# aptx4869lm/4DCapture-FPV

Hardware: AMD Instinct MI355X
Metric: frames/sec global-opt (fixed iters), 1024f clip/500k-pt scene; Chamfer GB/s (higher is better)
Workload: dtype f32; 1 GPU; BASELINE config 3: 1024-frame clip, 500000-pt scene, 500 contact verts, 500 Adam iterations (phase split 0.8), full loss; frames sharded over 1 GPU(s); frames=1024, scene_points=500000, contact_verts=500, iters=500, body_verts=10475, lbs_weights_per_vertex=4

## Files before the change

4dcapture-fpv_amd/csrc/fdc_chamfer.h:

```cpp
#pragma once
#include <hip/hip_runtime.h>
#include <stdlib.h>

#include <atomic>

#include "fdc_forms.h"
#include "fdc_math.h"

namespace fdc {

constexpr int NN_TILE = 1024;

struct NNTarget {
    const float4* pts;
    int n;
    const float4* bounds;
    const float4* sbounds;
    const float4* qbounds;
    const int* inv_perm;
    const uint4* frags;
    const float4* centers;
};


// ... 966 lines not shown
    scan(bc);
    if (T.centers) {
        float bm = INFINITY;
        int bc2 = -1;
        auto centre = [&](int c) {
            const float4 cc = T.centers[c];
            const float dx = x - cc.x, dy = y - cc.y, dz = z - cc.z;
            const float m = __builtin_amdgcn_sqrtf(fmaf(dz, dz, fmaf(dy, dy, dx * dx))) + cc.w;
            if (m < bm) { bm = m; bc2 = c; }
        };
        if (T.sbounds) {
            const int nsuper = (nchunk + ST4_SUPER - 1) / ST4_SUPER;
            for (int sb = 0; sb < nsuper; ++sb) {
                if (!(box_d2(T.sbounds[2 * sb], T.sbounds[2 * sb + 1], x, y, z) < bm * bm)) continue;
                for (int c = sb * ST4_SUPER; c < min(nchunk, (sb + 1) * ST4_SUPER); ++c) centre(c);
            }
        } else
            for (int c = 0; c < nchunk; ++c) centre(c);
        if (bc2 >= 0 && bc2 != bc && bm * bm < bd) scan(bc2);
    }
    seed[qi] = bi;
    seedpt[qi] = bp;
}

__global__ void nn_records_gather_kernel(const int* __restrict__ idx, int nq, const float4* __restrict__ scene, const int* __restrict__ inv_perm,
                                         float4* __restrict__ seedpt) {
    const int qi = blockIdx.x * blockDim.x + threadIdx.x;
    if (qi >= nq) return;
    const int j = idx[qi];
    if (j < 0) return;
    const float4 p = scene[j];
    seedpt[qi] = make_float4(p.x, p.y, p.z, __int_as_float(inv_perm[j]));
}

__global__ void nn_combine_kernel(const float* __restrict__ pd, const int* __restrict__ pi, int nsplit, int nq,
                                  float* __restrict__ dist, int* __restrict__ idx) {
    int qi = blockIdx.x * blockDim.x + threadIdx.x;
    if (qi >= nq) return;
    float best = INFINITY;
    int bi = -1;
    for (int s = 0; s < nsplit; ++s) {
        float d = pd[(size_t)s * nq + qi];
        int j = pi[(size_t)s * nq + qi];
        if (j >= 0 && (bi < 0 || nn_better(d, j, best, bi))) { best = d; bi = j; }
    }
    dist[qi] = best;
    idx[qi] = bi;
}

__global__ void pack_points_kernel(const float* __restrict__ xyz, int n, float4* __restrict__ out) {
    int i = blockIdx.x * blockDim.x + threadIdx.x;
    if (i >= n) return;
    out[i] = make_float4(xyz[3 * (size_t)i], xyz[3 * (size_t)i + 1], xyz[3 * (size_t)i + 2], __int_as_float(i));
}

__global__ void pack_points_batched_kernel(const float* __restrict__ xyz, long long stride, int n, float4* __restrict__ out) {
    int i = blockIdx.x * blockDim.x + threadIdx.x;
    if (i >= n) return;
    const float* const p = xyz + (size_t)blockIdx.y * stride + 3 * (size_t)i;
    out[(size_t)blockIdx.y * n + i] = make_float4(p[0], p[1], p[2], __int_as_float(i));
}
__global__ void nn_combine_batched_kernel(const float* __restrict__ pd, const int* __restrict__ pi, int nsplit, int nq,
                                          float* __restrict__ dist, int* __restrict__ idx) {
    int qi = blockIdx.x * blockDim.x + threadIdx.x;
    if (qi >= nq) return;
    const size_t bb = blockIdx.y;
    pd += bb * nsplit * nq; pi += bb * nsplit * nq;
    float best = INFINITY;
    int bi = -1;
    for (int s = 0; s < nsplit; ++s) {
        float d = pd[(size_t)s * nq + qi];
        int j = pi[(size_t)s * nq + qi];
        if (j >= 0 && (bi < 0 || nn_better(d, j, best, bi))) { best = d; bi = j; }
    }
    dist[bb * nq + qi] = best;
    idx[bb * nq + qi] = bi;
}

__global__ void nn_grad_kernel(const float* __restrict__ q, const float4* __restrict__ tgt, const float* __restrict__ g,
                               const int* __restrict__ idx, int nq, float* __restrict__ gq) {
    int qi = blockIdx.x * blockDim.x + threadIdx.x;
    if (qi >= nq) return;
    int j = idx[qi];
    float gg = 2.f * g[qi];
    float4 p = j >= 0 ? tgt[j] : make_float4(0, 0, 0, 0);
    gq[3 * (size_t)qi] = j >= 0 ? gg * (q[3 * (size_t)qi] - p.x) : 0.f;
    gq[3 * (size_t)qi + 1] = j >= 0 ? gg * (q[3 * (size_t)qi + 1] - p.y) : 0.f;
    gq[3 * (size_t)qi + 2] = j >= 0 ? gg * (q[3 * (size_t)qi + 2] - p.z) : 0.f;
}

inline std::atomic<int>& nn_mode_ref() {
    static std::atomic<int> mode{0};
    return mode;
}

__global__ __launch_bounds__(1024) void nn_order_kernel(const int* __restrict__ work, int n, const int* __restrict__ prev,
                                                        int* __restrict__ order) {
    __shared__ int cnt[16][256], base[256];
    const int tid = threadIdx.x, w = tid >> 6;
    for (int e = tid; e < 16 * 256; e += 1024) (&cnt[0][0])[e] = 0;
    __syncthreads();
    for (int i = tid; i < n; i += 1024) atomicAdd(&cnt[w][255 - min(max(work[i], 0), 255)], 1);
    __syncthreads();
    if (tid < 256) {
        int run = 0;
        for (int k = 0; k < 16; ++k) { const int t = cnt[k][tid]; cnt[k][tid] = run; run += t; }
        base[tid] = run;
    }
    __syncthreads();
    if (tid < 64) {
        const int a = base[4 * tid], b = base[4 * tid + 1], c = base[4 * tid + 2], d = base[4 * tid + 3];
        int s = a + b + c + d, incl = s;
        for (int off = 1; off < 64; off <<= 1) { const int t = __shfl_up(incl, off, 64); if (tid >= off) incl += t; }
        const int ex = incl - s;
        base[4 * tid] = ex; base[4 * tid + 1] = ex + a; base[4 * tid + 2] = ex + a + b; base[4 * tid + 3] = ex + a + b + c;
    }
    __syncthreads();
    for (int i = tid; i < n; i += 1024) {
        const int k = 255 - min(max(work[i], 0), 255);
        order[base[k] + atomicAdd(&cnt[w][k], 1)] = prev ? prev[i] : i;
    }
}
struct NNOrder {
    bool on = false;
    int sorted_groups = 0;
    int cur = 0;
    int age = 0;
    int every = 32;
    int* qbuf = nullptr;
    int perm_n = 0;
    int perm_mode = 0;
    int n_kept = 0, n_permuted = 0, n_rebuilds = 0;
    int n_box[4] = {0, 0, 0, 0};
};
static inline size_t nn_query_order_ints(int nq);
static inline hipError_t nn_query_order(const float4* seedpt, int nq, int* qbuf, int* hdr, int groups, hipStream_t st);

static inline NNCache nn_stream_args(const NNCache* cache, NNOrder* ord, int groups, int wpg, int nq, const int* seed, const int* idx,
                                     const float4* seedpt, bool seed_missing) {
    NNCache nc = cache ? *cache : NNCache{nullptr, nullptr, nullptr, 0.f};
    const bool ordered = ord != nullptr && ord->on && nc.hdr != nullptr && ord->every > 0 && wpg == 1;
    nc.order_mode = !ordered ? 0 : (ord->sorted_groups == groups ? 2 + ord->cur : 1);
    const bool qorder = ordered && ord->qbuf != nullptr && ord->perm_mode != 1;
    nc.perm = qorder && ord->perm_n == nq ? ord->qbuf : nullptr;
    nc.keep = nc.keep && wpg == 1 && seedpt != nullptr && seed != nullptr && seed == idx && !seed_missing;
    if (ord) { ord->n_kept += nc.keep ? 1 : 0; ord->n_permuted += nc.perm ? 1 : 0; }
    if (ord && wpg == 1) ++ord->n_box[nc.box_lanes == 2 ? 1 : nc.box_lanes == 4 ? 2 : nc.box_lanes == 8 ? 3 : 0];
    return nc;
}
static inline hipError_t nn_stream_upkeep(const NNCache& nc, NNOrder* ord, int groups, int wpg, int nq, const float4* seedpt, bool seed_missing,
                                          hipStream_t st) {
    const bool ordered = ord != nullptr && ord->on && nc.hdr != nullptr && ord->every > 0 && wpg == 1;
    const bool qorder = ordered && ord->qbuf != nullptr && ord->perm_mode != 1;
    const bool resort = ordered && (ord->sorted_groups != groups || ++ord->age >= ord->every);
    if (qorder && ord->perm_mode == 0 && (ord->perm_n != nq || seed_missing || (resort && ord->sorted_groups == groups))) {
        const hipError_t e = nn_query_order(seedpt, nq, ord->qbuf, nc.hdr, groups, st);
        if (e != hipSuccess) return e;
        ord->perm_n = nq;
        ord->sorted_groups = 0;
        ord->age = 0;
        ++ord->n_rebuilds;
    } else if (resort) {
        const bool had = nc.order_mode >= 2;
        const int nxt = had ? 1 - ord->cur : 0;
        hipLaunchKernelGGL(nn_order_kernel, dim3(1), dim3(1024), 0, st, (const int*)(nc.hdr + 4 * groups), groups,
                           had ? (const int*)(nc.hdr + (5 + ord->cur) * groups) : (const int*)nullptr, nc.hdr + (5 + nxt) * groups);
        ord->cur = nxt;
        ord->sorted_groups = groups;
        ord->age = 0;
    }
    return hipSuccess;
}

static inline hipError_t nn_search(const float* q, int nq, const NNTarget& T, float* dist, int* idx, float* pd, int* pi,
                                   int nsplit, hipStream_t st, const int* seed = nullptr, bool seed_missing = false,
                                   float4* seedpt = nullptr, bool* seedpt_written = nullptr, const NNCache* cache = nullptr,
                                   NNOrder* ord = nullptr) {
    if (seedpt_written) *seedpt_written = false;
    if (nq <= 0) return hipSuccess;
    const NNPlan pl = plan_nn_search(nq, T.n, seed != nullptr && T.bounds != nullptr, T.frags != nullptr, seedpt != nullptr && seed == idx, nsplit,
                                     nn_mode_ref(), proc_switches());
    const dim3 grid(pl.grid), block(pl.block);
    note_form(form_name(pl.form));
    if (pl.wpg) {
        if (seed_missing)
            hipLaunchKernelGGL(nn_seed_kernel, dim3((nq + 255) / 256), dim3(256), 0, st, q, nq, T, idx, seedpt);
        if (seedpt_written) *seedpt_written = true;
        {
            const int groups = pl.groups, wpg = pl.wpg;
            const NNCache nc = nn_stream_args(cache, ord, groups, wpg, nq, seed, idx, seedpt, seed_missing);
            if (wpg == 4) hipLaunchKernelGGL((nn_stream4_kernel<4>), grid, block, 0, st, q, nq, T, seed, seedpt, dist, idx, nc, NNNoSegs{});
            else if (wpg == 2) hipLaunchKernelGGL((nn_stream4_kernel<2>), grid, block, 0, st, q, nq, T, seed, seedpt, dist, idx, nc, NNNoSegs{});
            else hipLaunchKernelGGL((nn_stream4_kernel<1, 1>), grid, block, 0, st, q, nq, T, seed, seedpt, dist, idx, nc, NNNoSegs{});
            const hipError_t e = nn_stream_upkeep(nc, ord, groups, wpg, nq, seedpt, seed_missing, st);
            if (e != hipSuccess) return e;
        }
        return hipGetLastError();
    }
    if (pl.form == F_NN_MFMA && pl.nq_blocks == 2) hipLaunchKernelGGL((nn_mfma_kernel<2>), grid, block, 0, st, q, nq, T, nsplit, seed, pd, pi, 0LL, 0LL);
    else if (pl.form == F_NN_MFMA) hipLaunchKernelGGL((nn_mfma_kernel<4>), grid, block, 0, st, q, nq, T, nsplit, seed, pd, pi, 0LL, 0LL);
    else hipLaunchKernelGGL((nn_direct_kernel<2>), grid, block, 0, st, q, nq, T, nsplit, pd, pi, 0LL, 0LL);
    hipLaunchKernelGGL(nn_combine_kernel, dim3((nq + 255) / 256), dim3(256), 0, st, pd, pi, nsplit, nq, dist, idx);
    return hipGetLastError();
}

struct NNSegSearch { const float* q; int nq; NNTarget T; float* dist; int* idx; float4* seedpt; NNCache cache; NNOrder* ord; bool seed_missing; };
static inline hipError_t nn_search_segments(const NNSegPlan& pl, const NNSegSearch* sg, int nseg, hipStream_t st) {
    if (!pl.one_launch || nseg < 1 || nseg > NN_MAX_SEGS || pl.grid_y != nseg) return hipErrorInvalidValue;
    note_form(pl.name);
    NNSegs a{};
    for (int s = 0; s < nseg; ++s) {
        const NNSegSearch& g = sg[s];
        const int groups = (g.nq + 31) / 32;
        if (g.nq <= 0 || groups > pl.grid_x) return hipErrorInvalidValue;
        if (g.seed_missing)
            hipLaunchKernelGGL(nn_seed_kernel, dim3((g.nq + 255) / 256), dim3(256), 0, st, g.q, g.nq, g.T, g.idx, g.seedpt);
        NNSeg& d = a.s[s];
        d.q = g.q; d.nq = g.nq; d.groups = groups; d.T = g.T; d.idx = g.idx; d.seedpt = g.seedpt; d.dist = g.dist;
        d.cache = nn_stream_args(&g.cache, g.ord, groups, 1, g.nq, g.idx, g.idx, g.seedpt, g.seed_missing);
    }
    hipLaunchKernelGGL((nn_stream4_kernel<1, 1, true>), dim3(pl.grid_x, nseg), dim3(pl.block), 0, st, (const float*)nullptr, 0, NNTarget{},
                       (const int*)nullptr, (float4*)nullptr, (float*)nullptr, (int*)nullptr, NNCache{nullptr, nullptr, nullptr, 0.f}, a);
    for (int s = 0; s < nseg; ++s) {
        const NNSegSearch& g = sg[s];
        const hipError_t e = nn_stream_upkeep(a.s[s].cache, g.ord, a.s[s].groups, 1, g.nq, g.seedpt, g.seed_missing, st);
        if (e != hipSuccess) return e;
    }
    return hipGetLastError();
}

static inline hipError_t nn_search_batched(const NNBatchPlan& pl, const float* q, long long qs, int nq, const float* tgt, long long ts, int nt,
                                           int B, float4* pk, float* dist, int* idx, float* pd, int* pi, hipStream_t st) {
    note_form(pl.name);
    const long long pks = ts == 0 ? 0 : nt;
    for (int b0 = 0; b0 < B; b0 += NN_MAX_GRID_Y) {
        const int nb = std::min(B - b0, NN_MAX_GRID_Y);
        const float* const qb = q + (size_t)b0 * qs;
        float4* const pkb = pk + (size_t)b0 * pks;
        float* const pdb = pd + (size_t)b0 * pl.nsplit * nq;
        int* const pib = pi + (size_t)b0 * pl.nsplit * nq;
        if (ts != 0 || b0 == 0)
            hipLaunchKernelGGL(pack_points_batched_kernel, dim3((nt + 255) / 256, ts == 0 ? 1 : nb), dim3(256), 0, st, tgt + (size_t)b0 * ts, ts, nt, pkb);
        const NNTarget T{pkb, nt, nullptr, nullptr, nullptr, nullptr, nullptr, nullptr};
        const dim3 grid(pl.grid_x, nb), block(pl.block);
        if (pl.mfma) hipLaunchKernelGGL((nn_mfma_kernel<4, true>), grid, block, 0, st, qb, nq, T, pl.nsplit, (const int*)nullptr, pdb, pib, qs, pks);
        else hipLaunchKernelGGL((nn_direct_kernel<2, true>), grid, block, 0, st, qb, nq, T, pl.nsplit, pdb, pib, qs, pks);
        hipLaunchKernelGGL(nn_combine_batched_kernel, dim3((nq + 255) / 256, nb), dim3(256), 0, st, pdb, pib, pl.nsplit, nq,
                           dist + (size_t)b0 * nq, idx + (size_t)b0 * nq);
    }
    return hipGetLastError();
}

}
```

4dcapture-fpv_amd/csrc/fdc_chamfer_bwd.h:

```cpp
#pragma once
#include <hip/hip_runtime.h>

#include "fdc_scene.h"

namespace fdc {

static_assert(SC_RS_TILE == QS_TILE, "the histogram and the scatter kernel cut the keys into the same tiles");

constexpr long long CB_MAX_SORT = 0x7fffffffLL - 2 * QS_TILE;

static inline int cb_blocks(long long n) { return (int)((n + QS_TILE - 1) / QS_TILE); }
static inline int cb_passes(unsigned maxkey) { int p = 1; while (p < 4 && (maxkey >> (8 * p)) != 0u) ++p; return p; }
static inline size_t cb_key_words(long long n) { return 2 * (size_t)n + 256 * (size_t)cb_blocks(n) + 256; }

__global__ __launch_bounds__(256) void cb_keys_kernel(const int* __restrict__ idx, int total, int cnt, int ndest, int per_batch,
                                                      unsigned invalid, unsigned* __restrict__ key, int* __restrict__ val) {
    const long long p = (long long)blockIdx.x * 256 + threadIdx.x;
    if (p >= total) return;
    const int j = idx[p];
    const unsigned b = (unsigned)(p / cnt);
    key[p] = (j >= 0 && j < ndest) ? (per_batch ? b * (unsigned)ndest + (unsigned)j : (unsigned)j) : invalid;
    val[p] = (int)p;
}

static inline hipError_t cb_group(const int* idx, int B, int cnt, int ndest, bool per_batch, unsigned* key, int* val, unsigned* hist,
                                  hipStream_t st, int* buf) {
    const int total = B * cnt, nb = cb_blocks(total);
    const unsigned invalid = per_batch ? (unsigned)B * (unsigned)ndest : (unsigned)ndest;
    unsigned* const tot = hist + 256 * (size_t)nb;
    hipLaunchKernelGGL(cb_keys_kernel, dim3((total + 255) / 256), dim3(256), 0, st, idx, total, cnt, ndest, per_batch ? 1 : 0, invalid, key, val);
    const int passes = cb_passes(invalid);
    for (int pass = 0; pass < passes; ++pass) {
        const size_t a = (size_t)(pass & 1) * total, b = (size_t)((pass & 1) ^ 1) * total;
        hipLaunchKernelGGL(sc_rs_hist_kernel, dim3(nb), dim3(256), 0, st, key + a, total, 8 * pass, hist, nb);
        hipLaunchKernelGGL(nn_qs_rows_kernel, dim3(64), dim3(256), 0, st, hist, nb, tot);
        hipLaunchKernelGGL(nn_qs_scatter_kernel, dim3(nb), dim3(256), 0, st, key + a, val + a, key + b, val + b, total, 8 * pass, hist, tot, nb);
    }
    *buf = passes & 1;
    return hipGetLastError();
}

struct CbSide {
    const float* xo; long long so;
    const float* xs; long long ss;
    int B, no, nsrc;
    const float* g_own; const int* idx_own;
    const float* g_src;
    int reduce;
};
__device__ __forceinline__ void cb_own_term(const CbSide& c, int b0, int d, float acc[3]) {
#pragma clang fp contract(off)
    acc[0] = acc[1] = acc[2] = 0.f;
    if (c.g_own == nullptr) return;
    const int b1 = c.reduce ? c.B : b0 + 1;
    for (int b = b0; b < b1; ++b) {
        const size_t p = (size_t)b * c.no + d;
        const int j = c.idx_own[p];
        if (j < 0 || j >= c.nsrc) continue;
        const float gg = 2.f * c.g_own[p];
        const float* const po = c.xo + (size_t)b * c.so + 3 * (size_t)d;
        const float* const ps = c.xs + (size_t)b * c.ss + 3 * (size_t)j;
#pragma unroll
        for (int k = 0; k < 3; ++k) {
            const float v = gg * (po[k] - ps[k]);
            acc[k] = c.reduce ? acc[k] + v : v;
        }
    }
}
__device__ __forceinline__ void cb_add_term(const CbSide& c, int p, int d, float S[3]) {
#pragma clang fp contract(off)
    const int b = p / c.nsrc, i = p - b * c.nsrc;
    const float gg = 2.f * c.g_src[p];
    const float* const po = c.xo + (size_t)b * c.so + 3 * (size_t)d;
    const float* const ps = c.xs + (size_t)b * c.ss + 3 * (size_t)i;
#pragma unroll
    for (int k = 0; k < 3; ++k) { const float v = gg * (ps[k] - po[k]); S[k] = S[k] + v; }
}
__device__ __forceinline__ void cb_store(float* __restrict__ out, size_t t, const float acc[3], const float S[3]) {
#pragma clang fp contract(off)
#pragma unroll
    for (int k = 0; k < 3; ++k) out[3 * t + k] = acc[k] - S[k];
}

__global__ __launch_bounds__(256) void cb_gather_kernel(CbSide c, const unsigned* __restrict__ skey, const int* __restrict__ sval, int nsorted,
                                                        float* __restrict__ out) {
    const long long t = (long long)blockIdx.x * 256 + threadIdx.x;
    const long long ndest = c.reduce ? (long long)c.no : (long long)c.B * c.no;
    if (t >= ndest) return;
    const int b0 = (int)((unsigned)t / (unsigned)c.no), d = (int)((unsigned)t - (unsigned)b0 * (unsigned)c.no);
    float acc[3], S[3] = {0.f, 0.f, 0.f};
    cb_own_term(c, b0, d, acc);
    if (skey != nullptr) {
        const unsigned want = (unsigned)t;
        int lo = 0, hi = nsorted;
        while (lo < hi) {
            const int mid = lo + ((hi - lo) >> 1);
            if (skey[mid] < want) lo = mid + 1; else hi = mid;
        }
        for (int s = lo; s < nsorted && skey[s] == want; ++s) cb_add_term(c, sval[s], d, S);
    }
    cb_store(out, (size_t)t, acc, S);
}

}
```

4dcapture-fpv_amd/csrc/fdc_forms.h:

```cpp
#pragma once
#include <stddef.h>
#include <stdlib.h>

#include <algorithm>

#include "fdc_clips.h"

#if defined(__HIPCC__)
#define FDC_FORMS_HD __host__ __device__
#else
#define FDC_FORMS_HD
#endif

namespace fdc {

struct FormSwitches {
    int clip_fwd_rows = 336;
    int clip_kgrad_rows = 257;
    int pn_rb2 = 1;
    int pn_nw = 0;
    bool pn_ksw = true;
    bool gemm_split3 = true;
    int nn_stream = -2;
    bool nn_seed = true, nn_cull = true;
// ... 97 lines not shown
    size_t lds = 0;
    size_t max_lds = 0;
    PnMap mp = {};
    bool two_partials = false;
};

inline PanelPlan plan_panel3(int M, int K, int ntile, int nst, int np, const FormSwitches& sw) {
    PanelPlan p;
    const int kpad = (K + 31) & ~31;
    if (kpad > PN3_MAX_K) return p;
    const size_t b_bytes = pn_b_bytes(np, ntile, nst);
    if (b_bytes > (size_t)(16u << 20) && M >= 32 && kpad <= 768) {
        const int nrb = (M + 31) / 32, ncb = (ntile + 7) / 8, cpg = (ncb + 7) / 8;
        p.form = F_PANEL3_WIDE;
        p.cs = std::max(1, std::min(cpg, (256 + 8 * nrb - 1) / (8 * nrb)));
        p.grid = 8 * nrb * p.cs; p.block = 512; p.lds = pn_lds_bytes(np, kpad, 2);
        return p;
    }
    if ((sw.pn_rb2 == 1 || sw.pn_rb2 == 2) && M >= sw.clip_fwd_rows && kpad <= 768 && ntile >= 48) {
        p.form = F_PANEL3_RB2;
        p.grid = 8 * ((M + 31) / 32); p.block = 768; p.lds = pn_lds_bytes(np, kpad, 2);
        return p;
    }
    const int nrb = (M + 15) / 16;
    p.form = F_PANEL3;
    p.nw = 8;
    if (nrb * ((ntile + 7) / 8) < 128 && nrb * ((ntile + 3) / 4) >= 128) p.nw = 4;
    if (sw.pn_nw == 8 || sw.pn_nw == 4 || sw.pn_nw == 2) p.nw = sw.pn_nw;
    p.mp = panel_map(nrb, (ntile + p.nw - 1) / p.nw, (size_t)M * K * 4, b_bytes);
    p.grid = 8 * p.mp.rpg * p.mp.cpg; p.block = 64 * p.nw; p.lds = pn_lds_bytes(np, kpad, 1);
    return p;
}

inline PanelPlan plan_blend_backward(int M, int K, int ntile, int nst, int np, bool may_split, const FormSwitches& sw) {
    PanelPlan p;
    const int kpad = (K + 31) & ~31, nst_all = (K + 31) >> 5;
    if (may_split && (sw.pn_rb2 == 1 || sw.pn_rb2 == 3) && M >= sw.clip_kgrad_rows && ntile <= 32 && nst_all >= 2 &&
        32 * ((nst_all + 1) / 2) <= 768) {
        p.form = F_PANEL3_RB2K;
        p.two_partials = true;
        p.grid = 8 * ((M + 31) / 32); p.block = 512; p.lds = pn_lds_bytes(np, 32 * ((nst_all + 1) / 2), 2);
        return p;
    }
    constexpr int kmin = 1664;
    const bool big_k = (M >= 384 && K >= kmin) || (M >= 192 && K >= kmin + 240);
    if (!big_k && sw.pn_ksw && kpad <= PN3_MAX_K && kpad >= 768 && ((M + 15) / 16) * ((ntile + 7) / 8) < 128) {
        const int nrb = (M + 15) / 16;
        p.form = F_PANEL3_KSW;
        p.T = (nrb * ((ntile + 1) / 2) >= 192 || nrb * ntile > 256) ? 2 : 1;
        p.mp = panel_map(nrb, (ntile + p.T - 1) / p.T, (size_t)M * K * 4, pn_b_bytes(np, ntile, nst));
        p.grid = 8 * p.mp.rpg * p.mp.cpg; p.block = 512; p.lds = pn_lds_bytes(np, kpad, 1);
        p.max_lds = pn_lds_bytes(np, PN3_MAX_K, 1);
        return p;
    }
    if (!big_k && panel_gemm3_fits(K)) return plan_panel3(M, K, ntile, nst, np, sw);
    constexpr int rb = PN3_KLOOP_RB, T = PN3_KLOOP_T;
    p.form = F_PANEL3_KLOOP;
    p.ks = panel_gemm3_kloop_parts(M, ntile);
    p.grid = p.ks * ((ntile + 8 * T - 1) / (8 * T)) * ((M + 16 * rb - 1) / (16 * rb)); p.block = 512;
    p.lds = pn_lds_bytes(np, 32 * PN3_KLOOP_SLAB, rb);
    p.max_lds = 150 * 1024;
    return p;
}

inline size_t blend_skin_lds_bytes(int np, int kfeat, int ja) {
    return pn_lds_bytes(np, (kfeat + 31) & ~31, 2) + (size_t)(32 * ja * 12 + 32 * 12 + 32 * 4 + 2 * 64 * 4 + 3 * 32 * 64) * sizeof(float);
}
struct ContactFwdPlan { Form form = F_SKIN_FWD; int grid = 0, grid_y = 1, block = 0; size_t lds = 0, max_lds = 0; };
inline ContactFwdPlan plan_contact_forward(int nl, int nc, int kfeat, int np, bool blend_done, bool permuted_panel, bool vpack, int K, int ja_hi,
                                           const FormSwitches& sw) {
    ContactFwdPlan p;
    if (!blend_done && sw.fuse_skin && sw.gemm_split3 && permuted_panel && vpack && K <= 4 && nl >= sw.clip_fwd_rows &&
        blend_skin_lds_bytes(np, kfeat, ja_hi) <= (size_t)150 * 1024) {
        p.form = F_BLEND_SKIN_FWD;
        p.grid = 8 * ((nl + 31) / 32); p.block = 768; p.lds = blend_skin_lds_bytes(np, kfeat, ja_hi); p.max_lds = 150 * 1024;
        return p;
    }
    p.grid = (nc + 255) / 256; p.grid_y = nl; p.block = 256;
    return p;
}

constexpr int SKB_VCH = 1024;
constexpr int SKB_ROW = 6;
constexpr int SKS_MAXV = 1024, SKS_MAXNNZ = 6144;
struct SkinBwdPlan {
    Form form = F_NONE;
    int G = 0;
    int vpt = 0, kc = 0;
    int nch = 1;
    int grid = 0, block = 256;
    size_t lds = 0;
    bool ja_rows = false;
};
inline SkinBwdPlan plan_skin_bwd_any(int nrows, int nc, bool mfma_da) {
    SkinBwdPlan p;
    p.lds = mfma_da ? std::max((size_t)std::min(nc, SKB_VCH) * SKB_ROW, (size_t)4 * 64 * 16) * sizeof(float)
                    : (size_t)std::min(nc, SKB_VCH) * 12 * sizeof(float);
    p.grid = nrows;
    if (nc <= SKB_VCH) { p.form = F_SKIN_BWD_FRAME; return p; }
    p.nch = (nc + SKB_VCH - 1) / SKB_VCH;
    p.form = mfma_da ? F_SKIN_BWD_CHUNKS_MFMA : F_SKIN_BWD_CHUNKS_LIST;
    return p;
}
inline SkinBwdPlan plan_contact_skin_bwd(int nl, int nc, int nnz, int K, bool vpack, bool csc_v16, bool aligned16, bool mfma_da, bool skin_vec) {
    const size_t lds_small = (size_t)6 * nc * sizeof(float) + (size_t)nnz * sizeof(float) + (((size_t)nnz * 2 + 15) & ~(size_t)15);
    if (!(nc <= SKS_MAXV && nnz <= SKS_MAXNNZ && lds_small <= 57000)) return plan_skin_bwd_any(nl, nc, mfma_da);
    SkinBwdPlan p;
    p.grid = nl; p.lds = lds_small; p.ja_rows = true;
    const int G = (K + 3) / 4;
    const size_t ldsv = (size_t)9 * nc * sizeof(float) + (size_t)((nnz + 3) & ~3) * sizeof(float) + (size_t)((nnz + 7) & ~7) * 2;
    if (skin_vec && nc <= 512 && G <= 3 && nnz <= 2048 * G && ldsv <= 60000 && (nc & 3) == 0 && vpack && csc_v16 && aligned16) {
        p.form = F_SKIN_BWD_VEC; p.G = G; p.lds = ldsv;
        return p;
    }
    p.form = F_SKIN_BWD_SMALL;
    if (nc <= 512 && nnz <= 2048) { p.vpt = 2; p.kc = 8; }
    else if (nc <= 512) { p.form = F_SKIN_BWD_SMALL_K; p.vpt = 2; p.kc = 24; }
    else if (nnz <= 4096) { p.vpt = 4; p.kc = 16; }
    else { p.vpt = 4; p.kc = 24; }
    return p;
}

#ifndef FDC_MF_CH
#define FDC_MF_CH 512
#endif
constexpr int MF_CH = FDC_MF_CH;
constexpr int MF_MAXCHUNK = 2048;
constexpr FDC_FORMS_HD int nn_split_len(int nt, int nsplit) {
    return ((nt + nsplit - 1) / nsplit + MF_CH - 1) / MF_CH * MF_CH;
}
constexpr int nn_grid_blocks(int qblocks, int nsplit) { return (qblocks + 7) / 8 * 8 * nsplit; }
constexpr bool nn_use_mfma(int nq, int nt, int mode) { return mode == 1 ? false : mode == 2 ? true : (long long)nq * nt >= (1LL << 22); }
inline int nn_pick_nsplit(int nq, int nt, bool culled = false) {
    int qblocks = culled ? (nq + 255) / 256 : (nq + 511) / 512;
    int ns = 1;
    const int target = culled ? 1536 : 1024;
    while (qblocks * ns < target && ns < 64 && nt / (ns * 2) >= 4 * MF_CH) ns *= 2;
    if (!culled && qblocks >= 512 && nt >= 8 * MF_CH) ns = std::max(ns, 2);
    while (nn_split_len(nt, ns) / MF_CH > MF_MAXCHUNK) ns *= 2;
    return ns;
}
constexpr FDC_FORMS_HD int nn_box_lanes(int n, int forced) {
    return (forced == 2 || forced == 4 || forced == 8) ? forced : n <= 8 ? 8 : n <= 16 ? 4 : 2;
}
constexpr FDC_FORMS_HD unsigned long long nn_box_fold(unsigned long long hits, int lpb) {
    hits |= hits >> 1;
    if (lpb >= 4) hits |= hits >> 2;
    if (lpb >= 8) hits |= hits >> 4;
    return hits & (lpb == 2 ? 0x5555555555555555ull : lpb == 4 ? 0x1111111111111111ull : 0x0101010101010101ull);
}
FDC_FORMS_HD inline int nn_box_rank(unsigned long long folded, int lane) { return __builtin_popcountll(folded & ((1ull << lane) - 1ull)); }
FDC_FORMS_HD inline int nn_box_count(unsigned long long folded) { return __builtin_popcountll(folded); }

struct NNPlan {
    Form form = F_NN_DIRECT;
    int wpg = 0;
    int nq_blocks = 0;
    int groups = 0;
    int grid = 0, block = 256;
};
inline NNPlan plan_nn_search(int nq, int nt, bool culled, bool frags, bool seed_in_place, int nsplit, int mode, const FormSwitches& sw) {
    NNPlan p;
    const bool mfma = nn_use_mfma(nq, nt, mode);
    if (culled && frags && sw.nn_stream != 0 && mfma && seed_in_place && (nt + MF_CH - 1) / MF_CH <= 16384) {
        p.groups = (nq + 31) / 32;
        if (sw.nn_stream < 0) {
            p.wpg = p.groups >= 2816 ? 1 : p.groups >= 2304 ? 2 : 4;
        } else {
            p.wpg = (sw.nn_stream / 10 == 4) ? 4 : (sw.nn_stream / 10 == 2) ? 2 : 1;
        }
        const int wpb = p.wpg == 1 ? 1 : 4;
        p.form = p.wpg == 4 ? F_NN_STREAM_W4 : p.wpg == 2 ? F_NN_STREAM_W2 : F_NN_STREAM_W1;
        p.grid = ((p.groups * p.wpg + wpb - 1) / wpb + 7) / 8 * 8; p.block = 64 * wpb;
        return p;
    }
    if (mfma) { p.form = F_NN_MFMA; p.nq_blocks = culled ? 2 : 4; }
    p.grid = nn_grid_blocks(mfma && culled ? (nq + 255) / 256 : (nq + 511) / 512, nsplit);
    return p;
}

constexpr int NN_MAX_SEGS = 16;
struct NNSegPlan {
    bool one_launch = false;
    const char* name = nullptr;
    int grid_x = 0, grid_y = 0, block = 64;
};
inline NNSegPlan plan_nn_segments(int nseg, const int* seg_nq, const int* seg_nt, bool culled, bool frags, bool seed_in_place, int nsplit, int mode,
                                  const FormSwitches& sw) {
    NNSegPlan p;
    if (nseg < 2 || nseg > NN_MAX_SEGS || sw.nn_segments_loop) return p;
    int big = 0;
    for (int s = 0; s < nseg; ++s) {
        if (seg_nq[s] > seg_nq[big]) big = s;
        if (plan_nn_search(seg_nq[s], seg_nt[s], culled, frags, seed_in_place, nsplit, mode, sw).wpg == 0) return p;
    }
    const NNPlan pl = plan_nn_search(seg_nq[big], seg_nt[big], culled, frags, seed_in_place, nsplit, mode, sw);
    if (pl.form != F_NN_STREAM_W1) return p;
    p.one_launch = true;
    p.name = "nn_stream4_kernel(1 wave per group, segments)";
    p.grid_x = pl.grid; p.grid_y = nseg; p.block = pl.block;
    return p;
}

constexpr int NN_MAX_GRID_Y = 65535;
struct NNBatchPlan {
    bool mfma = false;
    const char* name = "nn_direct_batched";
    int nsplit = 1, qblocks = 1, grid_x = 1, block = 256;
    int launches = 1;
};
inline NNBatchPlan plan_nn_batched(int nq, int nt, int B, int mode) {
    NNBatchPlan p;
    p.mfma = nn_use_mfma(nq, nt, mode);
    p.name = p.mfma ? "nn_mfma_batched" : "nn_direct_batched";
    p.qblocks = (int)(((long long)nq + 511) / 512);
    const long long flat = std::min<long long>((long long)p.qblocks * 512 * B, 1LL << 30);
    p.nsplit = nn_pick_nsplit((int)flat, nt);
    p.grid_x = p.qblocks * p.nsplit;
    p.launches = (B + NN_MAX_GRID_Y - 1) / NN_MAX_GRID_Y;
    return p;
}

constexpr int POSE_NJ = 55, POSE_NJW = 23;
struct PoseJoints {
    int jn = POSE_NJ, jr = POSE_NJ, nlev = -1;
    bool world = true;
};
inline PoseJoints plan_pose_joints(const int* parents, const int* depth, int ja_hi, bool contact_state, bool need_world, bool trim = true) {
    PoseJoints p;
    p.nlev = 0;
    for (int j = 0; j < POSE_NJ; ++j) p.nlev = std::max(p.nlev, depth[j] + 1);
    if (!trim) return p;
    const int jn = std::min(POSE_NJ, std::max(1, std::max(contact_state ? ja_hi : 0, need_world ? POSE_NJW : 0)));
    if (jn == POSE_NJ) return p;
    for (int j = 0; j < jn; ++j) if (parents[j] >= j) return p;
    p.jn = jn;
    p.jr = contact_state ? POSE_NJ : jn;
    p.world = need_world;
    p.nlev = 0;
    for (int j = 0; j < jn; ++j) p.nlev = std::max(p.nlev, depth[j] + 1);
    return p;
}

inline Form plan_decoder(bool gemm_split3) { return gemm_split3 ? F_VPOSER_SPLIT : F_VPOSER_FP32; }

}
```

4dcapture-fpv_amd/csrc/fdc_scene.h:

```cpp
#pragma once
#include <hip/hip_runtime.h>

#include <algorithm>
#include <utility>
#include <vector>

#include "fdc_chamfer.h"

namespace fdc {

constexpr int SC_RS_ROUNDS = 16;
constexpr int SC_RS_TILE = 256 * SC_RS_ROUNDS;
constexpr int SC_SCAN_BATCH = 16;
constexpr int SC_PT_TILE = 1024;
constexpr int SC_SUPER = 16;

__device__ __forceinline__ unsigned sc_key(float v) {
    unsigned u = __float_as_uint(v);
    if ((u << 1) == 0u) u = 0u;
    return (u & 0x80000000u) ? ~u : (u | 0x80000000u);
}

__global__ __launch_bounds__(256) void sc_keys_kernel(const float* __restrict__ xyz, int n, int axis, unsigned* __restrict__ keys,
                                                      int* __restrict__ vals) {
    const int i = blockIdx.x * 256 + threadIdx.x;
    if (i < n) { keys[i] = sc_key(xyz[3 * (size_t)i + axis]); vals[i] = i; }
}

__global__ __launch_bounds__(256) void sc_rs_hist_kernel(const unsigned* __restrict__ keys, int n, int shift, unsigned* __restrict__ hist, int nb) {
    __shared__ unsigned h[256];
    h[threadIdx.x] = 0;
    __syncthreads();
    const int base = blockIdx.x * SC_RS_TILE;
    for (int r = 0; r < SC_RS_ROUNDS; ++r) {
        const int i = base + r * 256 + threadIdx.x;
        if (i < n) atomicAdd(&h[(keys[i] >> shift) & 255u], 1u);
    }
    __syncthreads();
    hist[(size_t)threadIdx.x * nb + blockIdx.x] = h[threadIdx.x];
}

__global__ __launch_bounds__(1024) void sc_scan_kernel(unsigned* __restrict__ a, int m) {
    __shared__ unsigned part[1024];
    a += (size_t)blockIdx.x * m;
    const int per = (m + 1023) / 1024;
    const int lo = min(m, (int)threadIdx.x * per), hi = min(m, lo + per);
    unsigned s = 0;
    for (int i0 = lo; i0 < hi; i0 += SC_SCAN_BATCH) {
        unsigned v[SC_SCAN_BATCH];
#pragma unroll
        for (int k = 0; k < SC_SCAN_BATCH; ++k) v[k] = i0 + k < hi ? a[i0 + k] : 0u;
#pragma unroll
        for (int k = 0; k < SC_SCAN_BATCH; ++k) s += v[k];
    }
    part[threadIdx.x] = s;
    __syncthreads();
    for (int o = 1; o < 1024; o <<= 1) {
        unsigned t = threadIdx.x >= (unsigned)o ? part[threadIdx.x - o] : 0u;
        __syncthreads();
        part[threadIdx.x] += t;
        __syncthreads();
    }
    unsigned run = part[threadIdx.x] - s;
    for (int i0 = lo; i0 < hi; i0 += SC_SCAN_BATCH) {
        unsigned v[SC_SCAN_BATCH];
#pragma unroll
        for (int k = 0; k < SC_SCAN_BATCH; ++k) v[k] = i0 + k < hi ? a[i0 + k] : 0u;
#pragma unroll
        for (int k = 0; k < SC_SCAN_BATCH; ++k)
            if (i0 + k < hi) { a[i0 + k] = run; run += v[k]; }
    }
}

__global__ __launch_bounds__(256) void sc_rs_scatter_kernel(const unsigned* __restrict__ kin, const int* __restrict__ vin,
                                                            unsigned* __restrict__ kout, int* __restrict__ vout, int n, int shift,
                                                            const unsigned* __restrict__ hist, int nb) {
    __shared__ unsigned base[256];
    __shared__ unsigned wcnt[4][256];
    const int tid = threadIdx.x, wave = tid >> 6, lane = tid & 63;
    base[tid] = hist[(size_t)tid * nb + blockIdx.x];
    const int tile0 = blockIdx.x * SC_RS_TILE;
    for (int r = 0; r < SC_RS_ROUNDS; ++r) {
        const int i = tile0 + r * 256 + tid;
        const bool valid = i < n;
        const unsigned key = valid ? kin[i] : 0u;
        const int val = valid ? vin[i] : 0;
        const unsigned d = (key >> shift) & 255u;
        unsigned long long m = __ballot(valid);
#pragma unroll
        for (int b = 0; b < 8; ++b) {
            const bool bit = (d >> b) & 1u;
            const unsigned long long bal = __ballot(bit);
            m &= bit ? bal : ~bal;
        }
        const int rank = __popcll(m & ((1ull << lane) - 1ull));
        for (int k = 0; k < 4; ++k) wcnt[k][tid] = 0;
        __syncthreads();
        if (valid && rank == 0) wcnt[wave][d] = (unsigned)__popcll(m);
        __syncthreads();
        if (valid) {
            unsigned off = base[d];
            for (int k = 0; k < wave; ++k) off += wcnt[k][d];
            kout[off + rank] = key;
            vout[off + rank] = val;
        }
        __syncthreads();
        base[tid] += wcnt[0][tid] + wcnt[1][tid] + wcnt[2][tid] + wcnt[3][tid];
        __syncthreads();
    }
}

constexpr int QS_ROUNDS = 16;
constexpr int QS_TILE = 256 * QS_ROUNDS;
static inline int nn_query_order_blocks(int nq) { return (nq + QS_TILE - 1) / QS_TILE; }
static inline size_t nn_query_order_ints(int nq) { return 4 * (size_t)nq + 256 * (size_t)nn_query_order_blocks(nq) + 256; }

__global__ __launch_bounds__(256) void nn_qs_keys_kernel(const float4* __restrict__ seedpt, int nq, unsigned* __restrict__ key,
                                                         int* __restrict__ val, unsigned* __restrict__ hist, int nb,
                                                         int* __restrict__ hdr, int groups) {
    __shared__ unsigned h[256];
    const int tid = threadIdx.x;
    h[tid] = 0;
    __syncthreads();
    const int tile0 = blockIdx.x * QS_TILE;
    for (int r = 0; r < QS_ROUNDS; ++r) {
        const int i = tile0 + r * 256 + tid;
        if (i < nq) {
            const int pos = __float_as_int(seedpt[i].w);
            const unsigned k = pos >= 0 ? min((unsigned)pos >> 7, 0xFFFFu) : 0xFFFFu;
            key[i] = k;
            val[i] = i;
            atomicAdd(&h[k & 255u], 1u);
        }
    }
    const int ghi = blockIdx.x == gridDim.x - 1 ? groups : min(groups, tile0 + QS_TILE);
    for (int i = tile0 + tid; i < ghi; i += 256) hdr[i] = -1;
    __syncthreads();
    hist[(size_t)tid * nb + blockIdx.x] = h[tid];
}

__global__ __launch_bounds__(256) void nn_qs_hist_kernel(const unsigned* __restrict__ keys, int n, unsigned* __restrict__ hist, int nb) {
    __shared__ unsigned h[256];
    h[threadIdx.x] = 0;
    __syncthreads();
    const int tile0 = blockIdx.x * QS_TILE;
    for (int r = 0; r < QS_ROUNDS; ++r) {
        const int i = tile0 + r * 256 + threadIdx.x;
        if (i < n) atomicAdd(&h[(keys[i] >> 8) & 255u], 1u);
    }
    __syncthreads();
    hist[(size_t)threadIdx.x * nb + blockIdx.x] = h[threadIdx.x];
}

__global__ __launch_bounds__(256) void nn_qs_rows_kernel(unsigned* __restrict__ hist, int nb, unsigned* __restrict__ tot) {
    const int row = blockIdx.x * 4 + (threadIdx.x >> 6), lane = threadIdx.x & 63;
    unsigned* const a = hist + (size_t)row * nb;
    unsigned carry = 0;
    for (int j0 = 0; j0 < nb; j0 += 256) {
        unsigned v[4];
#pragma unroll
        for (int k = 0; k < 4; ++k) { const int j = j0 + 64 * k + lane; v[k] = j < nb ? a[j] : 0u; }
#pragma unroll
        for (int k = 0; k < 4; ++k) {
            unsigned s = v[k];
#pragma unroll
            for (int o = 1; o < 64; o <<= 1) { const unsigned t = __shfl_up(s, o); if (lane >= o) s += t; }
            const int j = j0 + 64 * k + lane;
            if (j < nb) a[j] = carry + s - v[k];
            carry += __shfl(s, 63);
        }
    }
    if (lane == 0) tot[row] = carry;
}

__global__ __launch_bounds__(256) void nn_qs_scatter_kernel(const unsigned* __restrict__ kin, const int* __restrict__ vin,
                                                            unsigned* __restrict__ kout, int* __restrict__ vout, int n, int shift,
                                                            const unsigned* __restrict__ hist, const unsigned* __restrict__ tot, int nb) {
    __shared__ unsigned base[256];
    __shared__ unsigned wcnt[4][256];
    __shared__ unsigned wtot[4];
    const int tid = threadIdx.x, wave = tid >> 6, lane = tid & 63;
    {
        const unsigned t = tot[tid];
        unsigned s = t;
#pragma unroll
        for (int o = 1; o < 64; o <<= 1) { const unsigned u = __shfl_up(s, o); if (lane >= o) s += u; }
        if (lane == 63) wtot[wave] = s;
        __syncthreads();
        unsigned off = s - t;
        for (int k = 0; k < wave; ++k) off += wtot[k];
        base[tid] = off + hist[(size_t)tid * nb + blockIdx.x];
    }
    const int tile0 = blockIdx.x * QS_TILE;
    for (int r = 0; r < QS_ROUNDS; ++r) {
        const int i = tile0 + r * 256 + tid;
        const bool valid = i < n;
        const unsigned key = valid ? kin[i] : 0u;
        const int val = valid ? vin[i] : 0;
        const unsigned d = (key >> shift) & 255u;
        unsigned long long m = __ballot(valid);
#pragma unroll
        for (int b = 0; b < 8; ++b) {
            const bool bit = (d >> b) & 1u;
            const unsigned long long bal = __ballot(bit);
            m &= bit ? bal : ~bal;
        }
        const int rank = __popcll(m & ((1ull << lane) - 1ull));
        for (int k = 0; k < 4; ++k) wcnt[k][tid] = 0;
        __syncthreads();
        if (valid && rank == 0) wcnt[wave][d] = (unsigned)__popcll(m);
        __syncthreads();
        if (valid) {
            unsigned off = base[d];
            for (int k = 0; k < wave; ++k) off += wcnt[k][d];
            kout[off + rank] = key;
            vout[off + rank] = val;
        }
        __syncthreads();
        base[tid] += wcnt[0][tid] + wcnt[1][tid] + wcnt[2][tid] + wcnt[3][tid];
        __syncthreads();
    }
}

static inline hipError_t nn_query_order(const float4* seedpt, int nq, int* qbuf, int* hdr, int groups, hipStream_t st) {
    const int nb = nn_query_order_blocks(nq);
    int* const perm = qbuf;
    int* const val = qbuf + nq;
    unsigned* const key = (unsigned*)(qbuf + 2 * (size_t)nq);
    unsigned* const hist = key + 2 * (size_t)nq;
    unsigned* const tot = hist + 256 * (size_t)nb;
    hipLaunchKernelGGL(nn_qs_keys_kernel, dim3(nb), dim3(256), 0, st, seedpt, nq, key, perm, hist, nb, hdr, groups);
    hipLaunchKernelGGL(nn_qs_rows_kernel, dim3(64), dim3(256), 0, st, hist, nb, tot);
    hipLaunchKernelGGL(nn_qs_scatter_kernel, dim3(nb), dim3(256), 0, st, key, perm, key + nq, val, nq, 0, hist, tot, nb);
    hipLaunchKernelGGL(nn_qs_hist_kernel, dim3(nb), dim3(256), 0, st, key + nq, nq, hist, nb);
    hipLaunchKernelGGL(nn_qs_rows_kernel, dim3(64), dim3(256), 0, st, hist, nb, tot);
    hipLaunchKernelGGL(nn_qs_scatter_kernel, dim3(nb), dim3(256), 0, st, key + nq, val, key, perm, nq, 8, hist, tot, nb);
    return hipGetLastError();
}

__device__ __forceinline__ int sc_find_node(const int4* __restrict__ nodes, int nn, int p) {
    int lo = 0, hi = nn - 1;
    while (lo < hi) {
        const int mid = (lo + hi + 1) >> 1;
        if (nodes[mid].x <= p) lo = mid; else hi = mid - 1;
    }
    return lo;
}

__global__ __launch_bounds__(256) void sc_axis_kernel(const int4* __restrict__ nodes, int nn, const float* __restrict__ xyz,
                                                      const int* __restrict__ Lx, const int* __restrict__ Ly, const int* __restrict__ Lz,
                                                      unsigned char* __restrict__ axis) {
    const int i = blockIdx.x * 256 + threadIdx.x;
    if (i >= nn) return;
    const int4 nd = nodes[i];
    int ax = 0;
    if (nd.z < nd.y) {
        const int a = nd.x, b = nd.x + nd.y - 1;
        const float ex = xyz[3 * (size_t)Lx[b]] - xyz[3 * (size_t)Lx[a]];
        const float ey = xyz[3 * (size_t)Ly[b] + 1] - xyz[3 * (size_t)Ly[a] + 1];
        const float ez = xyz[3 * (size_t)Lz[b] + 2] - xyz[3 * (size_t)Lz[a] + 2];
        float best = ex;
        if (ey > best) { ax = 1; best = ey; }
        if (ez > best) { ax = 2; }
    }
    axis[i] = (unsigned char)ax;
}

__global__ __launch_bounds__(256) void sc_side_kernel(const int4* __restrict__ nodes, int nn, const unsigned char* __restrict__ axis,
                                                      const int* __restrict__ Lx, const int* __restrict__ Ly, const int* __restrict__ Lz,
                                                      int n, unsigned char* __restrict__ side) {
    const int p = blockIdx.x * 256 + threadIdx.x;
    if (p >= n) return;
    const int nd = sc_find_node(nodes, nn, p);
    const int4 d = nodes[nd];
    const int ax = axis[nd];
    const int id = (ax == 0 ? Lx : ax == 1 ? Ly : Lz)[p];
    side[id] = (unsigned char)((p - d.x) >= d.z);
}

struct ScLists { const int* in[4]; int* out[4]; };

__device__ __forceinline__ int sc_wave_incl_scan(int v) {
    const int lane = threadIdx.x & 63;
#pragma unroll
    for (int o = 1; o < 64; o <<= 1) { const int t = __shfl_up(v, o); if (lane >= o) v += t; }
    return v;
}

__global__ __launch_bounds__(256) void sc_part_count_kernel(ScLists L, const unsigned char* __restrict__ side, int n, unsigned* __restrict__ cnt, int nb) {
    __shared__ unsigned tot[4];
    if (threadIdx.x < 4) tot[threadIdx.x] = 0;
    __syncthreads();
    const int p0 = blockIdx.x * SC_PT_TILE + threadIdx.x * 4;
    for (int l = 0; l < 4; ++l) {
        int c = 0;
        for (int k = 0; k < 4; ++k) if (p0 + k < n) c += side[L.in[l][p0 + k]];
        const int s = sc_wave_incl_scan(c);
        if ((threadIdx.x & 63) == 63) atomicAdd(&tot[l], (unsigned)s);
    }
    __syncthreads();
    if (threadIdx.x < 4) cnt[(size_t)threadIdx.x * nb + blockIdx.x] = tot[threadIdx.x];
}

__global__ __launch_bounds__(256) void sc_part_scatter_kernel(ScLists L, const unsigned char* __restrict__ side, int n,
                                                              const int4* __restrict__ nodes, int nn, const unsigned* __restrict__ cnt, int nb) {
    __shared__ int wsum[4];
    const int tid = threadIdx.x, wave = tid >> 6;
    const int p0 = blockIdx.x * SC_PT_TILE + tid * 4;
    int4 nd[4];
    for (int k = 0; k < 4; ++k) nd[k] = nodes[sc_find_node(nodes, nn, min(p0 + k, n - 1))];
    for (int l = 0; l < 4; ++l) {
        int id[4], s[4], c = 0;
        for (int k = 0; k < 4; ++k) {
            id[k] = p0 + k < n ? L.in[l][p0 + k] : 0;
            s[k] = p0 + k < n ? side[id[k]] : 0;
            c += s[k];
        }
        const int inc = sc_wave_incl_scan(c);
        __syncthreads();
        if ((tid & 63) == 63) wsum[wave] = inc;
        __syncthreads();
        int ones = (int)cnt[(size_t)l * nb + blockIdx.x] + inc - c;
        for (int k = 0; k < wave; ++k) ones += wsum[k];
        for (int k = 0; k < 4; ++k) {
            const int p = p0 + k;
            if (p < n) {
                const int in_node = ones - nd[k].w;
                const int dst = s[k] ? nd[k].x + nd[k].z + in_node : nd[k].x + (p - nd[k].x - in_node);
                L.out[l][dst] = id[k];
            }
            ones += s[k];
        }
    }
}

__device__ __forceinline__ unsigned sc_bf16(float f) {
    unsigned u = __float_as_uint(f);
    u += 0x7FFFu + ((u >> 16) & 1u);
    return u >> 16;
}
__device__ __forceinline__ float sc_bf16f(unsigned h) { return __uint_as_float(h << 16); }
__device__ __forceinline__ float sc_pad(float lo, float hi) {
#pragma clang fp contract(off)
    return 1e-6f + 1e-6f * fmaxf(fabsf(lo), fabsf(hi));
}

__global__ __launch_bounds__(MF_CH) void sc_finalize_kernel(const float* __restrict__ xyz, const int* __restrict__ order, int n,
                                                            float4* __restrict__ orig, float4* __restrict__ sorted, int* __restrict__ inv,
                                                            float4* __restrict__ bounds, float4* __restrict__ qbounds,
                                                            uint4* __restrict__ frags, float4* __restrict__ centers) {
#pragma clang fp contract(off)
    static_assert(MF_CH % 256 == 0 && MF_CH / 4 % 64 == 0, "a quarter cell is a whole number of waves");
    constexpr int NW = MF_CH / 64, WPQ = NW / 4;
    __shared__ float wlo[NW][3], whi[NW][3], wr2[NW];
    __shared__ float cen[3];
    const int ch = blockIdx.x, j = threadIdx.x, wave = j >> 6, lane = j & 63;
    const int p = ch * MF_CH + j;
    const bool valid = p < n;
    float x = 0.f, y = 0.f, z = 0.f;
    int idx = 0;
    if (valid) {
        idx = order[p];
        x = xyz[3 * (size_t)idx]; y = xyz[3 * (size_t)idx + 1]; z = xyz[3 * (size_t)idx + 2];
        const float4 pt = make_float4(x, y, z, __int_as_float(idx));
        sorted[p] = pt;
        orig[idx] = pt;
        inv[idx] = p;
    }
    float lo[3] = {valid ? x : INFINITY, valid ? y : INFINITY, valid ? z : INFINITY};
    float hi[3] = {valid ? x : -INFINITY, valid ? y : -INFINITY, valid ? z : -INFINITY};
#pragma unroll
    for (int o = 32; o >= 1; o >>= 1)
        for (int k = 0; k < 3; ++k) { lo[k] = fminf(lo[k], __shfl_xor(lo[k], o)); hi[k] = fmaxf(hi[k], __shfl_xor(hi[k], o)); }
    if (lane == 0) for (int k = 0; k < 3; ++k) { wlo[wave][k] = lo[k]; whi[wave][k] = hi[k]; }
    __syncthreads();
    if (j < 4) {
        float ql[3], qh[3];
        for (int k = 0; k < 3; ++k) {
            ql[k] = INFINITY; qh[k] = -INFINITY;
            for (int w = 0; w < WPQ; ++w) { ql[k] = fminf(ql[k], wlo[j * WPQ + w][k]); qh[k] = fmaxf(qh[k], whi[j * WPQ + w][k]); }
        }
        if (ch * MF_CH + j * (MF_CH / 4) < n)
            for (int k = 0; k < 3; ++k) { const float pad = sc_pad(ql[k], qh[k]); ql[k] -= pad; qh[k] += pad; }
        else
            for (int k = 0; k < 3; ++k) qh[k] = INFINITY;
        qbounds[2 * ((size_t)ch * 4 + j)] = make_float4(ql[0], ql[1], ql[2], 0.f);
        qbounds[2 * ((size_t)ch * 4 + j) + 1] = make_float4(qh[0], qh[1], qh[2], 0.f);
    }
    if (j == 0) {
// ... 189 lines not shown
```

Measured before the change: 19190 frames/s.

## Grow query-reorder period after stable rebuilds and shorten sort tiles for small inputs

Once more than three query-order rebuilds have happened, the interval between NN query re-sorts now doubles, up to a cap of 128. The rebuild counter resets whenever seeds go missing. This cuts how often the radix sort of query keys runs during long optimizations. Separately, the radix-sort kernels are templated on rounds per block, and small query counts use 8 rounds so more blocks fill the GPU. The cost is a staler query ordering between sorts, which can hurt locality in the NN kernels.

```diff
diff --git a/4dcapture-fpv_amd/csrc/fdc_chamfer.h b/4dcapture-fpv_amd/csrc/fdc_chamfer.h
--- a/4dcapture-fpv_amd/csrc/fdc_chamfer.h
+++ b/4dcapture-fpv_amd/csrc/fdc_chamfer.h
@@ -1142,7 +1142,8 @@
                                           hipStream_t st) {
     const bool ordered = ord != nullptr && ord->on && nc.hdr != nullptr && ord->every > 0 && wpg == 1;
     const bool qorder = ordered && ord->qbuf != nullptr && ord->perm_mode != 1;
-    const bool resort = ordered && (ord->sorted_groups != groups || ++ord->age >= ord->every);
+    if (ord && seed_missing) ord->n_rebuilds = 0;
+    const bool resort = ordered && (ord->sorted_groups != groups || ++ord->age >= nn_order_period(ord->every, ord->n_rebuilds, nq));
     if (qorder && ord->perm_mode == 0 && (ord->perm_n != nq || seed_missing || (resort && ord->sorted_groups == groups))) {
         const hipError_t e = nn_query_order(seedpt, nq, ord->qbuf, nc.hdr, groups, st);
         if (e != hipSuccess) return e;
diff --git a/4dcapture-fpv_amd/csrc/fdc_chamfer_bwd.h b/4dcapture-fpv_amd/csrc/fdc_chamfer_bwd.h
--- a/4dcapture-fpv_amd/csrc/fdc_chamfer_bwd.h
+++ b/4dcapture-fpv_amd/csrc/fdc_chamfer_bwd.h
@@ -34,7 +34,7 @@
         const size_t a = (size_t)(pass & 1) * total, b = (size_t)((pass & 1) ^ 1) * total;
         hipLaunchKernelGGL(sc_rs_hist_kernel, dim3(nb), dim3(256), 0, st, key + a, total, 8 * pass, hist, nb);
         hipLaunchKernelGGL(nn_qs_rows_kernel, dim3(64), dim3(256), 0, st, hist, nb, tot);
-        hipLaunchKernelGGL(nn_qs_scatter_kernel, dim3(nb), dim3(256), 0, st, key + a, val + a, key + b, val + b, total, 8 * pass, hist, tot, nb);
+        hipLaunchKernelGGL((nn_qs_scatter_kernel<QS_ROUNDS>), dim3(nb), dim3(256), 0, st, key + a, val + a, key + b, val + b, total, 8 * pass, hist, tot, nb);
     }
     *buf = passes & 1;
     return hipGetLastError();
diff --git a/4dcapture-fpv_amd/csrc/fdc_forms.h b/4dcapture-fpv_amd/csrc/fdc_forms.h
--- a/4dcapture-fpv_amd/csrc/fdc_forms.h
+++ b/4dcapture-fpv_amd/csrc/fdc_forms.h
@@ -273,6 +273,18 @@
 FDC_FORMS_HD inline int nn_box_rank(unsigned long long folded, int lane) { return __builtin_popcountll(folded & ((1ull << lane) - 1ull)); }
 FDC_FORMS_HD inline int nn_box_count(unsigned long long folded) { return __builtin_popcountll(folded); }
 
+#ifndef FDC_NN_PERIOD_GROWTH
+#define FDC_NN_PERIOD_GROWTH 1
+#endif
+constexpr int NN_PERIOD_HOLD = 3, NN_PERIOD_MAX = 128, NN_PERIOD_GROW_MAX_QUERIES = 1 << 21;
+constexpr FDC_FORMS_HD int nn_order_period(int base, int rebuilds, int nq) {
+    if (base <= 0) return 0;
+    int p = base;
+    if (FDC_NN_PERIOD_GROWTH && nq <= NN_PERIOD_GROW_MAX_QUERIES)
+        for (int r = NN_PERIOD_HOLD; r < rebuilds && p < NN_PERIOD_MAX; ++r) p = 2 * p < NN_PERIOD_MAX ? 2 * p : NN_PERIOD_MAX;
+    return p;
+}
+
 struct NNPlan {
     Form form = F_NN_DIRECT;
     int wpg = 0;
diff --git a/4dcapture-fpv_amd/csrc/fdc_scene.h b/4dcapture-fpv_amd/csrc/fdc_scene.h
--- a/4dcapture-fpv_amd/csrc/fdc_scene.h
+++ b/4dcapture-fpv_amd/csrc/fdc_scene.h
@@ -112,18 +112,22 @@
 
 constexpr int QS_ROUNDS = 16;
 constexpr int QS_TILE = 256 * QS_ROUNDS;
-static inline int nn_query_order_blocks(int nq) { return (nq + QS_TILE - 1) / QS_TILE; }
+constexpr int QS_ROUNDS_SHORT = 8, QS_FILL_BLOCKS = 256;
+static inline int nn_query_order_rounds(int nq) { return (nq + QS_TILE - 1) / QS_TILE < QS_FILL_BLOCKS ? QS_ROUNDS_SHORT : QS_ROUNDS; }
+static inline int nn_query_order_blocks(int nq) { const int tile = 256 * nn_query_order_rounds(nq); return (nq + tile - 1) / tile; }
 static inline size_t nn_query_order_ints(int nq) { return 4 * (size_t)nq + 256 * (size_t)nn_query_order_blocks(nq) + 256; }
 
+template <int ROUNDS>
 __global__ __launch_bounds__(256) void nn_qs_keys_kernel(const float4* __restrict__ seedpt, int nq, unsigned* __restrict__ key,
                                                          int* __restrict__ val, unsigned* __restrict__ hist, int nb,
                                                          int* __restrict__ hdr, int groups) {
+    constexpr int TILE = 256 * ROUNDS;
     __shared__ unsigned h[256];
     const int tid = threadIdx.x;
     h[tid] = 0;
     __syncthreads();
-    const int tile0 = blockIdx.x * QS_TILE;
-    for (int r = 0; r < QS_ROUNDS; ++r) {
+    const int tile0 = blockIdx.x * TILE;
+    for (int r = 0; r < ROUNDS; ++r) {
         const int i = tile0 + r * 256 + tid;
         if (i < nq) {
             const int pos = __float_as_int(seedpt[i].w);
@@ -133,18 +137,19 @@
             atomicAdd(&h[k & 255u], 1u);
         }
     }
-    const int ghi = blockIdx.x == gridDim.x - 1 ? groups : min(groups, tile0 + QS_TILE);
+    const int ghi = blockIdx.x == gridDim.x - 1 ? groups : min(groups, tile0 + TILE);
     for (int i = tile0 + tid; i < ghi; i += 256) hdr[i] = -1;
     __syncthreads();
     hist[(size_t)tid * nb + blockIdx.x] = h[tid];
 }
 
+template <int ROUNDS>
 __global__ __launch_bounds__(256) void nn_qs_hist_kernel(const unsigned* __restrict__ keys, int n, unsigned* __restrict__ hist, int nb) {
     __shared__ unsigned h[256];
     h[threadIdx.x] = 0;
     __syncthreads();
-    const int tile0 = blockIdx.x * QS_TILE;
-    for (int r = 0; r < QS_ROUNDS; ++r) {
+    const int tile0 = blockIdx.x * (256 * ROUNDS);
+    for (int r = 0; r < ROUNDS; ++r) {
         const int i = tile0 + r * 256 + threadIdx.x;
         if (i < n) atomicAdd(&h[(keys[i] >> 8) & 255u], 1u);
     }
@@ -173,6 +178,7 @@
     if (lane == 0) tot[row] = carry;
 }
 
+template <int ROUNDS = QS_ROUNDS>
 __global__ __launch_bounds__(256) void nn_qs_scatter_kernel(const unsigned* __restrict__ kin, const int* __restrict__ vin,
                                                             unsigned* __restrict__ kout, int* __restrict__ vout, int n, int shift,
                                                             const unsigned* __restrict__ hist, const unsigned* __restrict__ tot, int nb) {
@@ -191,8 +197,8 @@
         for (int k = 0; k < wave; ++k) off += wtot[k];
         base[tid] = off + hist[(size_t)tid * nb + blockIdx.x];
     }
-    const int tile0 = blockIdx.x * QS_TILE;
-    for (int r = 0; r < QS_ROUNDS; ++r) {
+    const int tile0 = blockIdx.x * (256 * ROUNDS);
+    for (int r = 0; r < ROUNDS; ++r) {
         const int i = tile0 + r * 256 + tid;
         const bool valid = i < n;
         const unsigned key = valid ? kin[i] : 0u;
@@ -222,6 +228,16 @@
     }
 }
 
+template <int ROUNDS>
+static inline void nn_query_order_launches(const float4* seedpt, int nq, unsigned* key, int* perm, int* val, unsigned* hist, unsigned* tot, int nb,
+                                           int* hdr, int groups, hipStream_t st) {
+    hipLaunchKernelGGL((nn_qs_keys_kernel<ROUNDS>), dim3(nb), dim3(256), 0, st, seedpt, nq, key, perm, hist, nb, hdr, groups);
+    hipLaunchKernelGGL(nn_qs_rows_kernel, dim3(64), dim3(256), 0, st, hist, nb, tot);
+    hipLaunchKernelGGL((nn_qs_scatter_kernel<ROUNDS>), dim3(nb), dim3(256), 0, st, key, perm, key + nq, val, nq, 0, hist, tot, nb);
+    hipLaunchKernelGGL((nn_qs_hist_kernel<ROUNDS>), dim3(nb), dim3(256), 0, st, key + nq, nq, hist, nb);
+    hipLaunchKernelGGL(nn_qs_rows_kernel, dim3(64), dim3(256), 0, st, hist, nb, tot);
+    hipLaunchKernelGGL((nn_qs_scatter_kernel<ROUNDS>), dim3(nb), dim3(256), 0, st, key + nq, val, key, perm, nq, 8, hist, tot, nb);
+}
 static inline hipError_t nn_query_order(const float4* seedpt, int nq, int* qbuf, int* hdr, int groups, hipStream_t st) {
     const int nb = nn_query_order_blocks(nq);
     int* const perm = qbuf;
@@ -229,12 +245,8 @@
     unsigned* const key = (unsigned*)(qbuf + 2 * (size_t)nq);
     unsigned* const hist = key + 2 * (size_t)nq;
     unsigned* const tot = hist + 256 * (size_t)nb;
-    hipLaunchKernelGGL(nn_qs_keys_kernel, dim3(nb), dim3(256), 0, st, seedpt, nq, key, perm, hist, nb, hdr, groups);
-    hipLaunchKernelGGL(nn_qs_rows_kernel, dim3(64), dim3(256), 0, st, hist, nb, tot);
-    hipLaunchKernelGGL(nn_qs_scatter_kernel, dim3(nb), dim3(256), 0, st, key, perm, key + nq, val, nq, 0, hist, tot, nb);
-    hipLaunchKernelGGL(nn_qs_hist_kernel, dim3(nb), dim3(256), 0, st, key + nq, nq, hist, nb);
-    hipLaunchKernelGGL(nn_qs_rows_kernel, dim3(64), dim3(256), 0, st, hist, nb, tot);
-    hipLaunchKernelGGL(nn_qs_scatter_kernel, dim3(nb), dim3(256), 0, st, key + nq, val, key, perm, nq, 8, hist, tot, nb);
+    if (nn_query_order_rounds(nq) == QS_ROUNDS_SHORT) nn_query_order_launches<QS_ROUNDS_SHORT>(seedpt, nq, key, perm, val, hist, tot, nb, hdr, groups, st);
+    else nn_query_order_launches<QS_ROUNDS>(seedpt, nq, key, perm, val, hist, tot, nb, hdr, groups, st);
     return hipGetLastError();
 }
 
```

After: 19390 frames/s, median of 6. 1.01x the previous value.
